# MisterBourbaki/vector-quantization-by-ml

Measured on NVIDIA B200. Metric: vq_lookups_per_sec, higher is better.
Workload: dtype f16

## Files before the change

### vector-quantization-by-ml_b200/csrc/common.cuh

```cuda
#pragma once

#include <cuda_bf16.h>
#include <cuda_fp16.h>
#include <cuda_runtime.h>
#include <stdint.h>
#include <stdio.h>

#include "../../include/vqb.h"

namespace vqb {

void set_error(const char* fmt, ...);

#define VQB_CUDA_TRY(expr)                                                              \
  do {                                                                                  \
    cudaError_t _e = (expr);                                                            \
    if (_e != cudaSuccess) {                                                            \
      vqb::set_error("%s:%d: %s -> %s", __FILE__, __LINE__, #expr, cudaGetErrorString(_e)); \
      return VQB_ERR_CUDA;                                                              \
    }                                                                                   \
  } while (0)

#define VQB_REQUIRE(cond, code, ...)                                                    \
  do {                                                                                  \
// ... 136 lines not shown
#pragma unroll
  for (int i = 0; i < 4; ++i) {
    const float2 f = __half22float2(*reinterpret_cast<const __half2*>(&w[i]));
    o.v[2 * i] = f.x; o.v[2 * i + 1] = f.y;
  }
  return o;
}

template <typename T> struct Raw8 { uint4 r; };
template <> struct Raw8<float> { float4 a, b; };
template <typename T> __device__ __forceinline__ Raw8<T> load_raw8(const T* p) {
  Raw8<T> o; o.r = __ldg(reinterpret_cast<const uint4*>(p)); return o;
}
template <> __device__ __forceinline__ Raw8<float> load_raw8<float>(const float* p) {
  Raw8<float> o;
  o.a = __ldg(reinterpret_cast<const float4*>(p));
  o.b = __ldg(reinterpret_cast<const float4*>(p) + 1);
  return o;
}
__device__ __forceinline__ F8 raw_to_f8(const Raw8<float>& w) {
  F8 o; o.v[0] = w.a.x; o.v[1] = w.a.y; o.v[2] = w.a.z; o.v[3] = w.a.w; o.v[4] = w.b.x; o.v[5] = w.b.y; o.v[6] = w.b.z; o.v[7] = w.b.w;
  return o;
}
__device__ __forceinline__ F8 raw_to_f8(const Raw8<__nv_bfloat16>& w) {
  F8 o;
  o.v[0] = __uint_as_float(w.r.x << 16); o.v[1] = __uint_as_float(w.r.x & 0xffff0000u);
  o.v[2] = __uint_as_float(w.r.y << 16); o.v[3] = __uint_as_float(w.r.y & 0xffff0000u);
  o.v[4] = __uint_as_float(w.r.z << 16); o.v[5] = __uint_as_float(w.r.z & 0xffff0000u);
  o.v[6] = __uint_as_float(w.r.w << 16); o.v[7] = __uint_as_float(w.r.w & 0xffff0000u);
  return o;
}
__device__ __forceinline__ F8 raw_to_f8(const Raw8<__half>& w) {
  const uint32_t u[4] = {w.r.x, w.r.y, w.r.z, w.r.w};
  F8 o;
#pragma unroll
  for (int i = 0; i < 4; ++i) {
    const float2 f = __half22float2(*reinterpret_cast<const __half2*>(&u[i]));
    o.v[2 * i] = f.x; o.v[2 * i + 1] = f.y;
  }
  return o;
}

__device__ __forceinline__ float warp_sum(float v) {
#pragma unroll
  for (int o = 16; o > 0; o >>= 1) v += __shfl_xor_sync(0xffffffffu, v, o);
  return v;
}
__device__ __forceinline__ double warp_sum(double v) {
#pragma unroll
  for (int o = 16; o > 0; o >>= 1) v += __shfl_xor_sync(0xffffffffu, v, o);
  return v;
}

#define VQB_DISPATCH_DTYPE(dtype, T, ...)                                                    \
  switch (dtype) {                                                                           \
    case VQB_F32:  { using T = float;          __VA_ARGS__; break; }                          \
    case VQB_BF16: { using T = __nv_bfloat16;  __VA_ARGS__; break; }                          \
    case VQB_F16:  { using T = __half;         __VA_ARGS__; break; }                          \
    default: vqb::set_error("unknown latent dtype %d", (int)(dtype)); return VQB_ERR_INVALID; \
  }

inline int dtype_size(int dt) { return dt == VQB_F32 ? 4 : 2; }

int launch_prepare_latents(const void* x, int x_dtype, int64_t rows, int64_t rows_per_head, int d, int dp,
                           const float* chdr, __half* xb, float* xinv, float* xn2, __half* xaug, uint32_t* scal,
                           cudaStream_t st);
int launch_make_bias(const void* cache, const CacheLayout& CL, int64_t H, int K, int metric,
                     uint32_t* scal, float* bias, float* err, __half* caug, cudaStream_t st, int derive_dx_dp = 0);
int launch_sample_bound(const void* x, int x_dtype, int64_t rows, int d, uint32_t* scal, cudaStream_t st);
struct ConvArgs {
  const void* x = nullptr;
  int x_dtype = 0;
  int d = 0;
};
int launch_search_tc(const __half* xb, const float* xinv, const float* xn2, float tie, const __half* xaug,
                     const __half* cb, const __half* caug, const float* chdr, const float* bias, int aug_mode,
                     int64_t H, int64_t N, int K, int dp, void* cand, uint32_t* scal, bool timing, cudaStream_t st,
                     const ConvArgs& conv = ConvArgs());
int search_tc_aug_mode(int64_t N, int K, int metric);
int search_tc_conv_ok(int64_t N, int K, int d, int x_dtype, int aug_mode, int requested);

int launch_loss_finalize(const double* part, const long long* cntp, int nblocks, int d, float* loss_out,
                         cudaStream_t st);

__device__ __forceinline__ float clamp_row_scale(float& s, float two_q, float two_mq) {
  const float cap = 32768.f * two_q;
  if (s > cap) s = cap;
  const float a = s * two_mq;
  return a >= 5.9604645e-8f ? a : 0.f;
}

constexpr float kTieSlack = 5.0e-7f;
__device__ __forceinline__ float row_norm2_bound(float n2, float r2) {
  return (n2 + 2.f * sqrtf(n2 * r2) + r2) * 1.0001f;
}

constexpr float kSampleGuard = 1.125f;
__device__ __forceinline__ float dx_bound_16bit(float xmax, int dp, float two_mq) {
  const float inv_s = fmaxf(xmax * 1.220703125e-4f, two_mq * 3.0517578125e-5f);
  return sqrtf((float)dp) * 2.9802322e-8f * inv_s * 1.01f;
}

__device__ __forceinline__ float pow2_scale_bits(float m) {
  const uint32_t ef = (__float_as_uint(m) >> 23) & 0xffu;
  if (!(m > 0.f) || ef == 0xffu) return 1.f;
  int sh = 14 - ((int)ef - 126);
  if (sh > 100) sh = 100;
  if (sh < -100) sh = -100;
  return __uint_as_float((uint32_t)(127 + sh) << 23);
}
__device__ __forceinline__ float pow2_recip(float s) { return __uint_as_float(0x7F000000u - __float_as_uint(s)); }

__host__ __device__ inline float pow2_scale(float m) {
  if (!(m > 0.f) || !isfinite(m)) return 1.f;
  int e = ilogbf(m) + 1;
  int sh = 14 - e;
  if (sh > 100) sh = 100;
  if (sh < -100) sh = -100;
  return ldexpf(1.f, sh);
}

}
```

### vector-quantization-by-ml_b200/csrc/ema.cu

```cuda
#include "common.cuh"

namespace vqb {

constexpr int kChunkRows = 64;

struct EmaLayout {
  size_t off_counts;
  size_t off_cursor;
  size_t off_start;
  size_t off_scale;
  size_t off_acc;
  size_t zero_bytes;
  size_t off_sorted;
  size_t off_total;
  size_t off_table;
  size_t total;
};
constexpr int kSortBlocks = 148;
constexpr int kSortMaxK = 12288;
inline EmaLayout ema_layout(int64_t H, int64_t N, int K, int d) {
  EmaLayout L;
  size_t o = 0;
  L.off_counts = o; o += align_up((size_t)H * K * 4);
  L.off_cursor = o; o += align_up((size_t)H * K * 4);
// ... 34 lines not shown

__global__ void ema_hist_kernel(const int64_t* __restrict__ idx, const uint8_t* __restrict__ mask, int64_t N, int K,
                                uint32_t* __restrict__ counts) {
  const int h = blockIdx.y;
  const int64_t n = (int64_t)blockIdx.x * blockDim.x + threadIdx.x;
  if (n >= N) return;
  if (mask && !mask[n]) return;
  const int64_t k = idx[(int64_t)h * N + n];
  if (k >= 0 && k < K) atomicAdd(counts + (int64_t)h * K + k, 1u);
}

__global__ void ema_scan_kernel(const uint32_t* __restrict__ counts, int K, uint32_t* __restrict__ start) {
  const int h = blockIdx.x;
  const uint32_t* c = counts + (int64_t)h * K;
  uint32_t* s = start + (int64_t)h * (K + 1);
  __shared__ uint32_t wsum[32];
  __shared__ uint32_t carry;
  if (threadIdx.x == 0) carry = 0;
  __syncthreads();
  const int lane = threadIdx.x & 31, warp = threadIdx.x >> 5;
  for (int base = 0; base < K; base += 1024) {
    const int k = base + threadIdx.x;
    const uint32_t v = k < K ? c[k] : 0u;
    uint32_t inc = v;
#pragma unroll
    for (int o = 1; o < 32; o <<= 1) {
      const uint32_t t = __shfl_up_sync(0xffffffffu, inc, o);
      if (lane >= o) inc += t;
    }
    if (lane == 31) wsum[warp] = inc;
    __syncthreads();
    if (warp == 0) {
      uint32_t w = wsum[lane];
#pragma unroll
      for (int o = 1; o < 32; o <<= 1) {
        const uint32_t t = __shfl_up_sync(0xffffffffu, w, o);
        if (lane >= o) w += t;
      }
      wsum[lane] = w;
    }
    __syncthreads();
    const uint32_t before = carry + (warp ? wsum[warp - 1] : 0u) + inc - v;
    if (k < K) s[k] = before;
    __syncthreads();
    if (threadIdx.x == 1023) carry = before + v;
    __syncthreads();
  }
  if (threadIdx.x == 0) s[K] = carry;
}

__global__ void ema_place_kernel(const int64_t* __restrict__ idx, const uint8_t* __restrict__ mask, int64_t N, int K,
                                 const uint32_t* __restrict__ start, uint32_t* __restrict__ cursor,
                                 int* __restrict__ sorted) {
  const int h = blockIdx.y;
  const int64_t n = (int64_t)blockIdx.x * blockDim.x + threadIdx.x;
  if (n >= N) return;
  if (mask && !mask[n]) return;
  const int64_t k = idx[(int64_t)h * N + n];
  if (k < 0 || k >= K) return;
  const uint32_t pos = start[(int64_t)h * (K + 1) + k] + atomicAdd(cursor + (int64_t)h * K + k, 1u);
  sorted[(int64_t)h * N + pos] = (int)n;
}


__global__ void __launch_bounds__(1024)
sort_hist_kernel(const int64_t* __restrict__ idx, const uint8_t* __restrict__ mask, int64_t N, int K,
                 uint32_t* __restrict__ table) {
  extern __shared__ uint32_t s_cnt[];
  const int h = blockIdx.y, b = blockIdx.x, B = gridDim.x;
  for (int k = threadIdx.x; k < K; k += blockDim.x) s_cnt[k] = 0u;
  __syncthreads();
  const int64_t span = (N + B - 1) / B, r0 = (int64_t)b * span, r1 = r0 + span < N ? r0 + span : N;
  for (int64_t n = r0 + threadIdx.x; n < r1; n += blockDim.x) {
    if (mask && !mask[n]) continue;
    const int64_t k = idx[(int64_t)h * N + n];
    if (k >= 0 && k < K) atomicAdd(s_cnt + k, 1u);
  }
  __syncthreads();
  uint32_t* t = table + ((int64_t)h * B + b) * K;
  for (int k = threadIdx.x; k < K; k += blockDim.x) t[k] = s_cnt[k];
}

__global__ void __launch_bounds__(256)
sort_prefix_kernel(uint32_t* __restrict__ table, int B, int K, uint32_t* __restrict__ counts) {
  const int h = blockIdx.y;
  const int k = blockIdx.x * blockDim.x + threadIdx.x;
  if (k >= K) return;
  uint32_t* t = table + (int64_t)h * B * K + k;
  uint32_t v = 0u;
  int b = 0;
  for (; b + 8 <= B; b += 8) {
    uint32_t x[8];
#pragma unroll
    for (int u = 0; u < 8; ++u) x[u] = t[(int64_t)(b + u) * K];
#pragma unroll
    for (int u = 0; u < 8; ++u) { t[(int64_t)(b + u) * K] = v; v += x[u]; }
  }
  for (; b < B; ++b) { const uint32_t x = t[(int64_t)b * K]; t[(int64_t)b * K] = v; v += x; }
  counts[(int64_t)h * K + k] = v;
}

__global__ void __launch_bounds__(1024)
sort_place_kernel(const int64_t* __restrict__ idx, const uint8_t* __restrict__ mask, int64_t N, int K,
                  const uint32_t* __restrict__ start, const uint32_t* __restrict__ table, int* __restrict__ sorted) {
  extern __shared__ uint32_t s_cur[];
  const int h = blockIdx.y, b = blockIdx.x, B = gridDim.x;
  const uint32_t* t = table + ((int64_t)h * B + b) * K;
  const uint32_t* st = start + (int64_t)h * (K + 1);
  for (int k = threadIdx.x; k < K; k += blockDim.x) s_cur[k] = st[k] + t[k];
  __syncthreads();
  const int64_t span = (N + B - 1) / B, r0 = (int64_t)b * span, r1 = r0 + span < N ? r0 + span : N;
  for (int64_t n = r0 + threadIdx.x; n < r1; n += blockDim.x) {
    if (mask && !mask[n]) continue;
    const int64_t k = idx[(int64_t)h * N + n];
    if (k < 0 || k >= K) continue;
    sorted[(int64_t)h * N + atomicAdd(s_cur + k, 1u)] = (int)n;
  }
}

static int launch_code_sort(const int64_t* idx, const uint8_t* mask, int64_t H, int64_t N, int K, uint32_t* counts,
                            uint32_t* cursor, uint32_t* start, int* sorted, uint32_t* table, cudaStream_t st) {
  if (K <= kSortMaxK && table != nullptr && N >= 4096) {
    const dim3 g((unsigned)kSortBlocks, (unsigned)H);
    const size_t smem = (size_t)K * 4;
    sort_hist_kernel<<<g, 1024, smem, st>>>(idx, mask, N, K, table);
    VQB_LAUNCH_CHECK();
    sort_prefix_kernel<<<dim3((unsigned)((K + 255) / 256), (unsigned)H), 256, 0, st>>>(table, kSortBlocks, K, counts);
    VQB_LAUNCH_CHECK();
    ema_scan_kernel<<<(unsigned)H, 1024, 0, st>>>(counts, K, start);
    VQB_LAUNCH_CHECK();
    sort_place_kernel<<<g, 1024, smem, st>>>(idx, mask, N, K, start, table, sorted);
    VQB_LAUNCH_CHECK();
    return VQB_OK;
  }
  dim3 g1((unsigned)((N + 255) / 256), (unsigned)H);
  ema_hist_kernel<<<g1, 256, 0, st>>>(idx, mask, N, K, counts);
  VQB_LAUNCH_CHECK();
  ema_scan_kernel<<<(unsigned)H, 1024, 0, st>>>(counts, K, start);
  VQB_LAUNCH_CHECK();
  ema_place_kernel<<<g1, 256, 0, st>>>(idx, mask, N, K, start, cursor, sorted);
  VQB_LAUNCH_CHECK();
  return VQB_OK;
}

template <typename T>
__global__ void __launch_bounds__(256, 3)
ema_segsum_kernel(const T* __restrict__ x, const int64_t* __restrict__ idx, const int* __restrict__ sorted,
                  const uint32_t* __restrict__ start, int64_t N, int K, int d, const int* __restrict__ scale_p,
                  unsigned long long* __restrict__ acc) {
  const int h = blockIdx.y;
  const int lane = threadIdx.x & 31;
  const int64_t chunk = (int64_t)blockIdx.x * (blockDim.x >> 5) + (threadIdx.x >> 5);
  const int64_t total = start[(int64_t)h * (K + 1) + K];
  const int64_t p0 = chunk * kChunkRows;
  if (p0 >= total) return;
  const int64_t p1 = p0 + kChunkRows < total ? p0 + kChunkRows : total;
  const float scale = ldexpf(1.f, scale_p[0]);
  const T* xh = x + (int64_t)h * N * d;
  const int64_t* idxh = idx + (int64_t)h * N;
  const int* srt = sorted + (int64_t)h * N;
  unsigned long long* acch = acc + (int64_t)h * K * d;
  const bool vec = (d & 3) == 0;

  const int n = (int)(p1 - p0);
  const int r_lo = lane < n ? srt[p0 + lane] : 0;
  const int r_hi = lane + 32 < n ? srt[p0 + 32 + lane] : 0;
  const int k_lo = lane < n ? (int)idxh[r_lo] : -1;
  const int k_hi = lane + 32 < n ? (int)idxh[r_hi] : -1;

  if ((d & 7) == 0) {
    for (int c0 = 0; c0 < d; c0 += 256) {
      const int j = c0 + lane * 8;
      const bool on = j < d;
      long long a[8];
#pragma unroll
      for (int e = 0; e < 8; ++e) a[e] = 0;
      int cur = -1;
      for (int i0 = 0; i0 < n; i0 += 4) {
        F8 v[4];
        int kk[4];
#pragma unroll
        for (int u = 0; u < 4; ++u) {
          const int i = i0 + u;
          const int r = __shfl_sync(0xffffffffu, i < 32 ? r_lo : r_hi, i & 31);
          kk[u] = __shfl_sync(0xffffffffu, i < 32 ? k_lo : k_hi, i & 31);
          if (i < n && on) v[u] = load8<T>(xh + (int64_t)r * d + j);
          else {
#pragma unroll
            for (int e = 0; e < 8; ++e) v[u].v[e] = 0.f;
          }
        }
#pragma unroll
        for (int u = 0; u < 4; ++u) {
          if (i0 + u < n) {
            if (kk[u] != cur) {
              if (cur >= 0 && on) {
                unsigned long long* o = acch + (int64_t)cur * d + j;
#pragma unroll
                for (int e = 0; e < 8; ++e) if (a[e]) atomicAdd(o + e, (unsigned long long)a[e]);
              }
#pragma unroll
              for (int e = 0; e < 8; ++e) a[e] = 0;
              cur = kk[u];
            }
#pragma unroll
            for (int e = 0; e < 8; ++e) a[e] += __float2ll_rn(v[u].v[e] * scale);
          }
        }
      }
      if (cur >= 0 && on) {
        unsigned long long* o = acch + (int64_t)cur * d + j;
#pragma unroll
        for (int e = 0; e < 8; ++e) if (a[e]) atomicAdd(o + e, (unsigned long long)a[e]);
      }
    }
    return;
  }

  for (int c0 = 0; c0 < d; c0 += 128) {
    const int j = c0 + lane * 4;
    const bool on = j < d;
    long long a0 = 0, a1 = 0, a2 = 0, a3 = 0;
    int cur = -1;
    for (int i0 = 0; i0 < n; i0 += 4) {
      float4 v[4];
      int kk[4];
#pragma unroll
      for (int u = 0; u < 4; ++u) {
        const int i = i0 + u;
        const int r = __shfl_sync(0xffffffffu, i < 32 ? r_lo : r_hi, i & 31);
        kk[u] = __shfl_sync(0xffffffffu, i < 32 ? k_lo : k_hi, i & 31);
        v[u] = make_float4(0.f, 0.f, 0.f, 0.f);
        if (i < n && on) {
          const T* xr = xh + (int64_t)r * d + j;
          if (vec) v[u] = load4<T>(xr);
          else {
            v[u].x = to_f32<T>(xr[0]);
            v[u].y = j + 1 < d ? to_f32<T>(xr[1]) : 0.f;
            v[u].z = j + 2 < d ? to_f32<T>(xr[2]) : 0.f;
            v[u].w = j + 3 < d ? to_f32<T>(xr[3]) : 0.f;
          }
        }
      }
#pragma unroll
      for (int u = 0; u < 4; ++u) {
        if (i0 + u < n) {
          if (kk[u] != cur) {
            if (cur >= 0 && on) {
              unsigned long long* o = acch + (int64_t)cur * d + j;
              if (a0) atomicAdd(o + 0, (unsigned long long)a0);
              if (j + 1 < d && a1) atomicAdd(o + 1, (unsigned long long)a1);
              if (j + 2 < d && a2) atomicAdd(o + 2, (unsigned long long)a2);
              if (j + 3 < d && a3) atomicAdd(o + 3, (unsigned long long)a3);
            }
            a0 = a1 = a2 = a3 = 0;
            cur = kk[u];
          }
          a0 += __float2ll_rn(v[u].x * scale);
          a1 += __float2ll_rn(v[u].y * scale);
          a2 += __float2ll_rn(v[u].z * scale);
          a3 += __float2ll_rn(v[u].w * scale);
        }
      }
    }
    if (cur >= 0 && on) {
      unsigned long long* o = acch + (int64_t)cur * d + j;
      if (a0) atomicAdd(o + 0, (unsigned long long)a0);
      if (j + 1 < d && a1) atomicAdd(o + 1, (unsigned long long)a1);
      if (j + 2 < d && a2) atomicAdd(o + 2, (unsigned long long)a2);
      if (j + 3 < d && a3) atomicAdd(o + 3, (unsigned long long)a3);
    }
  }
}

__global__ void ema_finalize_kernel(const long long* __restrict__ acc, const uint32_t* __restrict__ counts,
                                    const int* __restrict__ scale_p, int64_t HK, int d, float* __restrict__ stats) {
  const int64_t i = (int64_t)blockIdx.x * blockDim.x + threadIdx.x;
  const int64_t n = HK * (d + 1);
  if (i >= n) return;
  const int64_t k = i / (d + 1);
  const int j = (int)(i - k * (d + 1));
  if (j == d) stats[i] = (float)counts[k];
  else stats[i] = (float)ldexp((double)acc[k * d + j], -scale_p[0]);
}


struct FusedScale { int s; int pad; int e; int P; };

__global__ void fused_scale_kernel(const float* __restrict__ bound2, const uint32_t* __restrict__ own_bound,
                                   int64_t rows, int two_terms, int* __restrict__ scale) {
  float b = bound2 ? (bound2[0] + bound2[1]) : __uint_as_float(own_bound[0]);
  if (!(b > 0.f) || !isfinite(b)) b = 1.f;
  int e;
  frexpf(b, &e);
  e += 1;
  if (e > 100) e = 100;
  if (e < -100) e = -100;
  int lr = 0;
  while (((int64_t)1 << lr) < rows + 1) ++lr;
  int P = 22;
  if (two_terms) { P = 62 - lr; if (P > 44) P = 44; }
  scale[0] = P - e;
  scale[2] = e;
  scale[3] = P;
}


constexpr int kFusedChunkRows = 128;

struct RvqExtra {
  float* out;
  float* res_out;
  float* q_level;
  __half* next_xb;
  float* next_xinv;
  float* next_xn2;
  __half* next_xaug;
  uint32_t* next_scal;
  const float* next_chdr;
  int first;
  int dp;
};

template <typename T, int NB, int TERMS, bool RVQ>
__global__ void __launch_bounds__(256, 2)
quantize_ema_kernel(const T* __restrict__ x, const float* __restrict__ cb, const int64_t* __restrict__ idx,
                    const int* __restrict__ sorted, const uint32_t* __restrict__ start, int64_t N, int K, int d,
                    int training, const int* __restrict__ scale_p, float* __restrict__ q,
                    float* __restrict__ loss_rows, unsigned long long* __restrict__ acc, const RvqExtra R) {
  constexpr int U0 = (sizeof(T) == 2 ? 8 : 4) / NB;
  constexpr int U = RVQ ? (U0 > 1 ? U0 / 2 : 1) : U0;
  const int h = blockIdx.y;
  const int lane = threadIdx.x & 31;
  const int64_t chunk = (int64_t)blockIdx.x * (blockDim.x >> 5) + (threadIdx.x >> 5);
  const int64_t total = start[(int64_t)h * (K + 1) + K];
  const int64_t p0 = chunk * kFusedChunkRows;
  if (p0 >= total) return;
  const int n = (int)((p0 + kFusedChunkRows < total ? p0 + kFusedChunkRows : total) - p0);
  const int lpr = NB == 1 ? d >> 3 : 32;
  const int rpi = 32 / lpr;
  const int grp = lane / lpr, gl = lane - grp * lpr;
  const int j = gl * 8;
  const int e = scale_p[2], P = scale_p[3];
  const float M1 = ldexpf(1.5f, e + 1);
  const float M2 = ldexpf(1.5f, e + 23 - P);
  const uint32_t M1b = __float_as_uint(M1), M2b = __float_as_uint(M2);
  const int shift = P - 22;
  const T* xh = x + (int64_t)h * N * d;
  const float* cbh = cb + (int64_t)h * K * d;
  const int64_t* idxh = idx + (int64_t)h * N;
  const int* srt = sorted + (int64_t)h * N;
  float* qh = q + (int64_t)h * N * d;
  unsigned long long* acch = acc + (int64_t)h * K * d;

  int rid[4], kid[4];
#pragma unroll
  for (int t = 0; t < 4; ++t) {
    rid[t] = lane + 32 * t < n ? srt[p0 + 32 * t + lane] : 0;
    kid[t] = lane + 32 * t < n ? (int)idxh[rid[t]] : -1;
  }

  uint32_t sh[NB][8], sl[NB][8];
  float c[NB][8];
#pragma unroll
  for (int b = 0; b < NB; ++b)
#pragma unroll
    for (int t = 0; t < 8; ++t) { sh[b][t] = 0u; sl[b][t] = 0u; c[b][t] = 0.f; }
  int cur = -1;
  uint32_t cnt = 0;
  float max_n2 = 0.f, max_r2 = 0.f;
// ... 86 lines not shown
              const float4 p0 = *reinterpret_cast<const float4*>(R.out + off), p1 = *(reinterpret_cast<const float4*>(R.out + off) + 1);
              const float pv[8] = {p0.x, p0.y, p0.z, p0.w, p1.x, p1.y, p1.z, p1.w};
#pragma unroll
              for (int t = 0; t < 8; ++t) acc8[t] = __fadd_rn(pv[t], o[t]);
            }
            *reinterpret_cast<float4*>(R.out + off) = make_float4(acc8[0], acc8[1], acc8[2], acc8[3]);
            *(reinterpret_cast<float4*>(R.out + off) + 1) = make_float4(acc8[4], acc8[5], acc8[6], acc8[7]);
            }
#pragma unroll
            for (int t = 0; t < 8; ++t) {
              rn[b].v[t] = __fsub_rn(v.v[t], o[t]);
              mabs = fmaxf(mabs, fabsf(rn[b].v[t]));
            }
            *reinterpret_cast<float4*>(R.res_out + off) = make_float4(rn[b].v[0], rn[b].v[1], rn[b].v[2], rn[b].v[3]);
            *(reinterpret_cast<float4*>(R.res_out + off) + 1) = make_float4(rn[b].v[4], rn[b].v[5], rn[b].v[6], rn[b].v[7]);
            if (R.q_level) {
              *reinterpret_cast<float4*>(R.q_level + off) = make_float4(o[0], o[1], o[2], o[3]);
              *(reinterpret_cast<float4*>(R.q_level + off) + 1) = make_float4(o[4], o[5], o[6], o[7]);
            }
          }
        }
      }
      if (RVQ && R.next_xb) {
        const bool live = kk[u] >= 0;
        for (int o2 = lpr >> 1; o2 > 0; o2 >>= 1) mabs = fmaxf(mabs, __shfl_xor_sync(0xffffffffu, mabs, o2));
        float s = pow2_scale_bits(mabs);
        const float a = clamp_row_scale(s, R.next_chdr[4], R.next_chdr[5]);
        const float is = pow2_recip(s);
        if (gl == 0 && live) {
          R.next_xinv[rr[u]] = a > 0.f ? is : -is;
          const uint32_t aa = (uint32_t)__half_as_ushort(__float2half_rn(a));
          *reinterpret_cast<uint4*>(R.next_xaug + (int64_t)rr[u] * 8) = make_uint4(aa | (aa << 16), aa, 0u, 0u);
        }
        float n2 = 0.f, r2 = 0.f;
#pragma unroll
        for (int b = 0; b < NB; ++b) {
          uint32_t pk[4];
#pragma unroll
          for (int t = 0; t < 4; ++t) {
            const float v0 = rn[b].v[2 * t], v1 = rn[b].v[2 * t + 1];
            const __half2 hh = __floats2half2_rn(v0 * s, v1 * s);
            const float2 f = __half22float2(hh);
            pk[t] = *reinterpret_cast<const uint32_t*>(&hh);
            const float b0 = f.x * is, b1 = f.y * is;
            n2 += b0 * b0 + b1 * b1;
            const float e0 = v0 - b0, e1 = v1 - b1;
            r2 += e0 * e0 + e1 * e1;
          }
          if (live)
            *reinterpret_cast<uint4*>(R.next_xb + (int64_t)rr[u] * R.dp + b * 256 + j) = make_uint4(pk[0], pk[1], pk[2], pk[3]);
        }
        for (int o2 = lpr >> 1; o2 > 0; o2 >>= 1) {
          n2 += __shfl_xor_sync(0xffffffffu, n2, o2);
          r2 += __shfl_xor_sync(0xffffffffu, r2, o2);
        }
        if (gl == 0 && live) R.next_xn2[rr[u]] = row_norm2_bound(n2, r2);
        max_n2 = fmaxf(max_n2, n2);
        max_r2 = fmaxf(max_r2, r2);
      }
      if (loss_rows) {
        for (int o2 = lpr >> 1; o2 > 0; o2 >>= 1) sq += __shfl_xor_sync(0xffffffffu, sq, o2);
        if (kk[u] >= 0 && gl == 0) loss_rows[(int64_t)h * N + rr[u]] = sq;
      }
    }
  }
  flush();
  if (RVQ && R.next_xb) {
#pragma unroll
    for (int o2 = 16; o2 > 0; o2 >>= 1) {
      max_n2 = fmaxf(max_n2, __shfl_xor_sync(0xffffffffu, max_n2, o2));
      max_r2 = fmaxf(max_r2, __shfl_xor_sync(0xffffffffu, max_r2, o2));
    }
    if (lane == 0) {
      const float infl = 1.f + (float)R.dp * 2.4e-7f;
      atomicMax(R.next_scal + 0, __float_as_uint(sqrtf(max_n2 * infl) * 1.00001f));
      atomicMax(R.next_scal + 1, __float_as_uint(sqrtf(max_r2 * infl) * 1.00001f));
      if (blockIdx.x == 0 && threadIdx.x == 0) R.next_scal[7] = __float_as_uint(R.next_chdr[4]);
    }
  }
}

__global__ void __launch_bounds__(256)
loss_rows_partial_kernel(const float* __restrict__ loss_rows, int64_t rows, int64_t span, double* __restrict__ part,
                         long long* __restrict__ cntp) {
  const int64_t r0 = (int64_t)blockIdx.x * span;
  const int64_t r1 = r0 + span < rows ? r0 + span : rows;
  double t = 0.0;
  for (int64_t r = r0 + threadIdx.x; r < r1; r += 256) t += (double)loss_rows[r];
  __shared__ double s[256];
  s[threadIdx.x] = t;
  __syncthreads();
  for (int o = 128; o > 0; o >>= 1) {
    if ((int)threadIdx.x < o) s[threadIdx.x] += s[threadIdx.x + o];
    __syncthreads();
  }
  if (threadIdx.x == 0) { part[blockIdx.x] = s[0]; cntp[blockIdx.x] = r1 > r0 ? r1 - r0 : 0; }
}

constexpr int kLossBlocks = 1024;
struct FusedLayout {
  EmaLayout E;
  size_t off_loss_rows;
  size_t off_part;
  size_t off_cnt;
  size_t total;
};
inline FusedLayout fused_layout(int64_t H, int64_t N, int K, int d) {
  FusedLayout L;
  L.E = ema_layout(H, N, K, d);
  size_t o = L.E.total;
  L.off_loss_rows = o; o += align_up((size_t)(H * N > 0 ? H * N : 1) * 4);
  L.off_part = o;      o += align_up((size_t)kLossBlocks * 8);
  L.off_cnt = o;       o += align_up((size_t)kLossBlocks * 8);
  L.total = o;
  return L;
}
inline bool fused_width_ok(int d) { return d == 512 || (d >= 8 && d <= 256 && (d & (d - 1)) == 0); }


constexpr int kMomentRows = 256;
template <typename T>
__global__ void __launch_bounds__(256)
column_moments_kernel(const T* __restrict__ x, const uint8_t* __restrict__ mask, int64_t N, int d,
                      double* __restrict__ out, long long* __restrict__ rows_used) {
  const int h = blockIdx.y;
  const int64_t r0 = (int64_t)blockIdx.x * kMomentRows;
  const int64_t r1 = r0 + kMomentRows < N ? r0 + kMomentRows : N;
  const T* xh = x + (int64_t)h * N * d;
  for (int c = threadIdx.x; c < d; c += blockDim.x) {
    double s = 0.0, ss = 0.0;
    for (int64_t r = r0; r < r1; ++r) {
      if (mask && !mask[r]) continue;
      const double v = (double)to_f32<T>(xh[r * d + c]);
      s += v;
      ss = fma(v, v, ss);
    }
    atomicAdd(out + ((int64_t)h * d + c) * 2, s);
    atomicAdd(out + ((int64_t)h * d + c) * 2 + 1, ss);
  }
  if (threadIdx.x == 0) {
    long long n = 0;
    for (int64_t r = r0; r < r1; ++r) n += (!mask || mask[r]) ? 1 : 0;
    atomicAdd(reinterpret_cast<unsigned long long*>(rows_used + h), (unsigned long long)n);
  }
}

__device__ __forceinline__ float torch_lerp(float a, float b, float w) {
  const float diff = b - a;
  return fabsf(w) < 0.5f ? fmaf(w, diff, a) : fmaf(w - 1.f, diff, b);
}

__global__ void ema_apply_counts_kernel(const float* __restrict__ stats, float* __restrict__ cluster_size, float w,
                                        int K, int d, float* __restrict__ total) {
  const int h = blockIdx.x;
  __shared__ double s[1024];
  double t = 0.0;
  for (int k = threadIdx.x; k < K; k += 1024) {
    const int64_t i = (int64_t)h * K + k;
    const float v = torch_lerp(cluster_size[i], stats[i * (d + 1) + d], w);
    cluster_size[i] = v;
    t += (double)v;
  }
  s[threadIdx.x] = t;
  __syncthreads();
  for (int o = 512; o > 0; o >>= 1) {
    if ((int)threadIdx.x < o) s[threadIdx.x] += s[threadIdx.x + o];
    __syncthreads();
  }
  if (threadIdx.x == 0) total[h] = (float)s[0];
}

__global__ void __launch_bounds__(256)
ema_apply_rows_kernel(const float* __restrict__ stats, const float* __restrict__ cluster_size,
                      float* __restrict__ embed_avg, float* __restrict__ embeddings, float w, float eps, float keps,
                      int l2, int64_t H, int K, int d, const float* __restrict__ total) {
  const int lane = threadIdx.x & 31;
  const int64_t row = (int64_t)blockIdx.x * (blockDim.x >> 5) + (threadIdx.x >> 5);
  if (row >= H * K) return;
  const int64_t h = row / K;
// ... 155 lines not shown
  return VQB_OK;
}

extern "C" int vqb_quantize_ema_supported(int d) { return fused_width_ok(d) ? 1 : 0; }

extern "C" size_t vqb_quantize_ema_workspace_bytes(int64_t H, int64_t N, int K, int d) {
  if (H <= 0 || N < 0 || K <= 0 || d <= 0) return 0;
  return fused_layout(H, N, K, d).total;
}

static int quantize_ema_impl(const void* x, int x_dtype, const float* codebook, const int64_t* idx,
                             const float* absmax_bound2, int training, int want_loss, float* q_out,
                             float* loss_out, float* stats, int64_t H, int64_t N, int K, int d, void* ws,
                             size_t ws_bytes, const RvqExtra* rvq, void* stream) {
  VQB_REQUIRE(x && codebook && idx && (q_out || rvq) && stats && ws, VQB_ERR_INVALID, "vqb_quantize_ema: null pointer");
  VQB_REQUIRE(H > 0 && N >= 0 && K > 0 && d > 0 && H < 65536, VQB_ERR_INVALID, "vqb_quantize_ema: bad shape");
  VQB_REQUIRE(N < (1ll << 31), VQB_ERR_UNSUPPORTED, "N must be < 2^31");
  VQB_REQUIRE(fused_width_ok(d), VQB_ERR_UNSUPPORTED, "vqb_quantize_ema: d=%d (need a power of two <= 256, or 512)", d);
  VQB_REQUIRE(!want_loss || loss_out, VQB_ERR_INVALID, "vqb_quantize_ema: loss_out is null");
  FusedLayout L = fused_layout(H, N, K, d);
  VQB_REQUIRE(ws_bytes >= L.total, VQB_ERR_WORKSPACE, "quantize_ema workspace too small: %zu < %zu", ws_bytes, L.total);
  cudaStream_t st = (cudaStream_t)stream;
  char* w = (char*)ws;
  uint32_t* counts = (uint32_t*)(w + L.E.off_counts);
  uint32_t* cursor = (uint32_t*)(w + L.E.off_cursor);
  uint32_t* start = (uint32_t*)(w + L.E.off_start);
  int* scale = (int*)(w + L.E.off_scale);
  long long* acc = (long long*)(w + L.E.off_acc);
  int* sorted = (int*)(w + L.E.off_sorted);
  float* loss_rows = want_loss ? (float*)(w + L.off_loss_rows) : nullptr;
  double* part = (double*)(w + L.off_part);
  long long* cntp = (long long*)(w + L.off_cnt);
  const int two_terms = x_dtype == VQB_F32 ? 1 : 0;
  VQB_CUDA_TRY(cudaMemsetAsync(w, 0, L.E.zero_bytes, st));
  if (N > 0) {
    if (!absmax_bound2) {
      VQB_DISPATCH_DTYPE(x_dtype, T,
        absmax_kernel<T><<<1184, 256, 0, st>>>((const T*)x, H * N * (int64_t)d, (uint32_t*)(scale + 1)));
      VQB_LAUNCH_CHECK();
    }
    fused_scale_kernel<<<1, 1, 0, st>>>(absmax_bound2, (const uint32_t*)(scale + 1), N, two_terms, scale);
    VQB_LAUNCH_CHECK();
    if (rvq && rvq->next_scal) VQB_CUDA_TRY(cudaMemsetAsync(rvq->next_scal, 0, 8, st));
    if (int rc = launch_code_sort(idx, nullptr, H, N, K, counts, cursor, start, sorted,
                                  K <= kSortMaxK ? (uint32_t*)(w + L.E.off_table) : nullptr, st)) return rc;
    const int64_t chunks = (N + kFusedChunkRows - 1) / kFusedChunkRows;
    dim3 g2((unsigned)((chunks + 7) / 8), (unsigned)H);
#define VQB_QE_LAUNCH(T, NB, TERMS)                                                                          \
    quantize_ema_kernel<T, NB, TERMS, false><<<g2, 256, 0, st>>>((const T*)x, codebook, idx, sorted, start, N, K, d, \
                                                                 training, scale, q_out, loss_rows,              \
                                                                 (unsigned long long*)acc, RvqExtra{})
    if (rvq) {
      if (d == 512)
        quantize_ema_kernel<float, 2, 2, true><<<g2, 256, 0, st>>>((const float*)x, codebook, idx, sorted, start, N, K, d,
                                                                   training, scale, nullptr, loss_rows,
                                                                   (unsigned long long*)acc, *rvq);
      else
        quantize_ema_kernel<float, 1, 2, true><<<g2, 256, 0, st>>>((const float*)x, codebook, idx, sorted, start, N, K, d,
                                                                   training, scale, nullptr, loss_rows,
                                                                   (unsigned long long*)acc, *rvq);
    } else if (d == 512) {
      if (x_dtype == VQB_F32) VQB_QE_LAUNCH(float, 2, 2);
      else if (x_dtype == VQB_BF16) VQB_QE_LAUNCH(__nv_bfloat16, 2, 1);
      else if (x_dtype == VQB_F16) VQB_QE_LAUNCH(__half, 2, 1);
      else { set_error("unknown latent dtype %d", x_dtype); return VQB_ERR_INVALID; }
    } else {
      if (x_dtype == VQB_F32) VQB_QE_LAUNCH(float, 1, 2);
      else if (x_dtype == VQB_BF16) VQB_QE_LAUNCH(__nv_bfloat16, 1, 1);
      else if (x_dtype == VQB_F16) VQB_QE_LAUNCH(__half, 1, 1);
      else { set_error("unknown latent dtype %d", x_dtype); return VQB_ERR_INVALID; }
    }
#undef VQB_QE_LAUNCH
    VQB_LAUNCH_CHECK();
  }
  const int64_t n = H * (int64_t)K * (d + 1);
  ema_finalize_kernel<<<(unsigned)((n + 255) / 256), 256, 0, st>>>(acc, counts, scale, H * (int64_t)K, d, stats);
  VQB_LAUNCH_CHECK();
  if (want_loss) {
    const int64_t rows = H * N;
    int nblocks = 0;
    if (rows > 0) {
      const int64_t span = (rows + kLossBlocks - 1) / kLossBlocks;
      nblocks = (int)((rows + span - 1) / span);
      loss_rows_partial_kernel<<<nblocks, 256, 0, st>>>(loss_rows, rows, span, part, cntp);
      VQB_LAUNCH_CHECK();
    }
    int rc = launch_loss_finalize(part, cntp, nblocks, d, loss_out, st);
    if (rc) return rc;
  }
  return VQB_OK;
}

extern "C" int vqb_quantize_ema(const void* x, int x_dtype, const float* codebook, const int64_t* idx,
                                const float* absmax_bound2, int training, int want_loss, float* q_out,
                                float* loss_out, float* stats, int64_t H, int64_t N, int K, int d, void* ws,
                                size_t ws_bytes, void* stream) {
  return quantize_ema_impl(x, x_dtype, codebook, idx, absmax_bound2, training, want_loss, q_out, loss_out, stats, H, N,
                           K, d, ws, ws_bytes, nullptr, stream);
}

extern "C" int vqb_rvq_level_ema_supported(int d) { return (d == 64 || d == 128 || d == 256 || d == 512) ? 1 : 0; }

extern "C" int vqb_rvq_level_ema(const float* residual_in, float* residual_out, const float* codebook,
                                 const int64_t* idx, const float* absmax_bound2, int training, int first_level,
                                 float* quantized_out, float* q_out, float* loss_out, float* stats, int64_t N, int K,
                                 int d, void* ws, size_t ws_bytes, void* next_ws, size_t next_ws_bytes,
                                 const void* next_cache, void* stream) {
  VQB_REQUIRE(residual_in && residual_out && loss_out, VQB_ERR_INVALID, "vqb_rvq_level_ema: null pointer");
  VQB_REQUIRE(vqb_rvq_level_ema_supported(d), VQB_ERR_UNSUPPORTED, "vqb_rvq_level_ema: d=%d (64, 128, 256 or 512)", d);
  VQB_REQUIRE(residual_in != residual_out, VQB_ERR_INVALID, "vqb_rvq_level_ema: rows are visited in code order, the "
              "residual cannot be updated in place");
  RvqExtra R = {};
  R.out = quantized_out; R.res_out = residual_out; R.q_level = q_out; R.first = first_level; R.dp = d_pad(d);
  if (next_ws) {
    VQB_REQUIRE(next_cache != nullptr, VQB_ERR_INVALID, "vqb_rvq_level_ema: next_ws needs next_cache");
    SearchLayout SL = search_layout(1, N, K, d);
    VQB_REQUIRE(next_ws_bytes >= SL.total, VQB_ERR_WORKSPACE, "next-level search workspace too small");
    R.next_xb = (__half*)((char*)next_ws + SL.off_xb);
    R.next_xaug = (__half*)((char*)next_ws + SL.off_xaug);
    R.next_xinv = (float*)((char*)next_ws + SL.off_xinv);
    R.next_xn2 = (float*)((char*)next_ws + SL.off_xn2);
    R.next_scal = (uint32_t*)((char*)next_ws + SL.off_scal);
    R.next_chdr = (const float*)((const char*)next_cache + cache_layout(1, K, d).off_hdr);
  }
  return quantize_ema_impl(residual_in, VQB_F32, codebook, idx, absmax_bound2, training, 1, nullptr, loss_out, stats, 1,
                           N, K, d, ws, ws_bytes, &R, stream);
}

extern "C" int vqb_ema_apply_counts(const float* stats, float* cluster_size, float weight, int64_t H, int K, int d,
                                    float* totals_out, void* stream) {
  VQB_REQUIRE(stats && cluster_size && totals_out, VQB_ERR_INVALID, "vqb_ema_apply_counts: null pointer");
  VQB_REQUIRE(H > 0 && K > 0 && d > 0, VQB_ERR_INVALID, "vqb_ema_apply_counts: bad shape");
  ema_apply_counts_kernel<<<(unsigned)H, 1024, 0, (cudaStream_t)stream>>>(stats, cluster_size, weight, K, d, totals_out);
  VQB_LAUNCH_CHECK();
  return VQB_OK;
}

extern "C" int vqb_ema_apply_rows(const float* stats, const float* cluster_size, float* embed_avg, float* embeddings,
                                  float weight, double eps, int64_t k_total, int l2norm, int64_t H, int K, int d,
                                  const float* totals, void* stream) {
  VQB_REQUIRE(stats && cluster_size && embed_avg && embeddings && totals, VQB_ERR_INVALID,
              "vqb_ema_apply_rows: null pointer");
  VQB_REQUIRE(H > 0 && K > 0 && d > 0 && k_total >= K, VQB_ERR_INVALID, "vqb_ema_apply_rows: bad shape");
  const int64_t rows = H * (int64_t)K;
  ema_apply_rows_kernel<<<(unsigned)((rows + 7) / 8), 256, 0, (cudaStream_t)stream>>>(
      stats, cluster_size, embed_avg, embeddings, weight, (float)eps, (float)((double)k_total * eps), l2norm, H, K, d,
      totals);
  VQB_LAUNCH_CHECK();
  return VQB_OK;
}

extern "C" int vqb_ema_apply(const float* stats, float* cluster_size, float* embed_avg, float* embeddings,
                             float weight, double eps, int l2norm, int64_t H, int K, int d, void* ws,
                             size_t ws_bytes, void* stream) {
  VQB_REQUIRE(ws != nullptr && ws_bytes >= (size_t)H * 4, VQB_ERR_WORKSPACE, "ema_apply workspace too small");
  int rc = vqb_ema_apply_counts(stats, cluster_size, weight, H, K, d, (float*)ws, stream);
  if (rc) return rc;
  return vqb_ema_apply_rows(stats, cluster_size, embed_avg, embeddings, weight, eps, K, l2norm, H, K, d,
                            (const float*)ws, stream);
}

extern "C" int vqb_expire_scatter(const void* x, int x_dtype, const int64_t* sample_rows, int64_t m, float threshold,
                                  float reset, int l2norm, float* cluster_size, float* embed_avg, float* embeddings,
                                  int64_t N, int K, int d, void* stream) {
  VQB_REQUIRE(x && cluster_size && embed_avg && embeddings, VQB_ERR_INVALID, "vqb_expire_scatter: null pointer");
  VQB_REQUIRE(m >= 0 && N > 0 && K > 0 && d > 0, VQB_ERR_INVALID, "vqb_expire_scatter: bad shape");
  if (m == 0) return VQB_OK;
  VQB_REQUIRE(sample_rows != nullptr, VQB_ERR_INVALID, "vqb_expire_scatter: sample_rows is null");
  VQB_DISPATCH_DTYPE(x_dtype, T,
    expire_scatter_kernel<T><<<1, 1024, 0, (cudaStream_t)stream>>>((const T*)x, sample_rows, m, threshold, reset,
                                                                  l2norm, cluster_size, embed_avg, embeddings, N, K, d));
// ... 36 lines not shown
```

### vector-quantization-by-ml_b200/csrc/gather.cu

```cuda
#include "common.cuh"

namespace vqb {

constexpr int kGatherThreads = 256;

struct GatherLayout {
  size_t off_part;
  size_t off_cnt;
  size_t total;
};
static int gather_grid(int64_t rows) {
  static int sms = 0;
  if (!sms) {
    int dev = 0;
    cudaGetDevice(&dev);
    cudaDeviceGetAttribute(&sms, cudaDevAttrMultiProcessorCount, dev);
    if (sms <= 0) sms = 148;
  }
  int64_t need = (rows + (kGatherThreads / 32) - 1) / (kGatherThreads / 32);
  int64_t cap = (int64_t)sms * 8;
  return (int)(need < cap ? (need > 0 ? need : 1) : cap);
}
static GatherLayout gather_layout() {
  GatherLayout L;
// ... 53 lines not shown
        if (kLoss) { sq = fmaf(df.x, df.x, sq); sq = fmaf(df.y, df.y, sq); sq = fmaf(df.z, df.z, sq); sq = fmaf(df.w, df.w, sq); }
      }
    } else {
      for (int j = lane; j < d; j += 32) {
        const float xv = to_f32<T>(xr[j]);
        const float cv = cr[j];
        const float df = __fsub_rn(cv, xv);
        qr[j] = training ? __fadd_rn(xv, df) : cv;
        if (kLoss) sq = fmaf(df, df, sq);
      }
    }
    if (kLoss && in_loss) { sqd += (double)sq; if (lane == 0) ++used; }
  }
  if (kLoss) {
    sqd = warp_sum(sqd);
    __shared__ double s_sq[kGatherThreads / 32];
    __shared__ long long s_n[kGatherThreads / 32];
    if (lane == 0) { s_sq[warp] = sqd; s_n[warp] = used; }
    __syncthreads();
    if (threadIdx.x == 0) {
      double t = 0.0;
      long long c = 0;
      for (int i = 0; i < wpb; ++i) { t += s_sq[i]; c += s_n[i]; }
      part[blockIdx.x] = t;
      cntp[blockIdx.x] = c;
    }
  }
}

template <typename T, bool kLoss>
__global__ void __launch_bounds__(kGatherThreads)
gather_st_loss_narrow_kernel(const T* __restrict__ x, const float* __restrict__ cb, const int64_t* __restrict__ idx,
                             const uint8_t* __restrict__ mask, int training, float* __restrict__ q, int64_t H,
                             int64_t N, int K, int d, double* __restrict__ part, long long* __restrict__ cntp) {
  const int lane = threadIdx.x & 31, warp = threadIdx.x >> 5;
  const int wpb = kGatherThreads / 32;
  const int lpr = d >> 3, rpi = 32 / lpr;
  const int grp = lane / lpr, j = (lane - grp * lpr) * 8;
  const int64_t rows = H * N;
  double sqd = 0.0;
  long long used = 0;
  for (int64_t row0 = ((int64_t)blockIdx.x * wpb + warp) * rpi; row0 < rows; row0 += (int64_t)gridDim.x * wpb * rpi) {
    const int64_t row = row0 + grp;
    if (row >= rows) continue;
    const int64_t h = row / N, n = row - h * N;
    const int64_t code = idx[row];
    const bool in_loss = mask == nullptr || mask[n] != 0;
    const F8 xv = load8<T>(x + row * (int64_t)d + j);
    const float* cr = cb + (h * K + code) * (int64_t)d + j;
    const float4 c0 = __ldg(reinterpret_cast<const float4*>(cr)), c1 = __ldg(reinterpret_cast<const float4*>(cr) + 1);
    const float cv[8] = {c0.x, c0.y, c0.z, c0.w, c1.x, c1.y, c1.z, c1.w};
    float o[8], sq = 0.f;
#pragma unroll
    for (int e = 0; e < 8; ++e) {
      const float df = __fsub_rn(cv[e], xv.v[e]);
      o[e] = training ? __fadd_rn(xv.v[e], df) : cv[e];
      if (kLoss) sq = fmaf(df, df, sq);
    }
    float* qr = q + row * (int64_t)d + j;
    __stcs(reinterpret_cast<float4*>(qr), make_float4(o[0], o[1], o[2], o[3]));
    __stcs(reinterpret_cast<float4*>(qr) + 1, make_float4(o[4], o[5], o[6], o[7]));
    if (kLoss && in_loss) { sqd += (double)sq; if (j == 0) ++used; }
  }
  if (kLoss) {
    sqd = warp_sum(sqd);
#pragma unroll
    for (int o2 = 16; o2 > 0; o2 >>= 1) used += __shfl_xor_sync(0xffffffffu, used, o2);
    __shared__ double s_sq[kGatherThreads / 32];
    __shared__ long long s_n[kGatherThreads / 32];
    if (lane == 0) { s_sq[warp] = sqd; s_n[warp] = used; }
    __syncthreads();
    if (threadIdx.x == 0) {
      double t = 0.0;
      long long c = 0;
      for (int i = 0; i < wpb; ++i) { t += s_sq[i]; c += s_n[i]; }
      part[blockIdx.x] = t;
      cntp[blockIdx.x] = c;
    }
  }
}

__global__ void loss_finalize_kernel(const double* __restrict__ part, const long long* __restrict__ cntp, int nblocks,
                                     int d, float* __restrict__ loss_out) {
  __shared__ double s[256];
  __shared__ long long c[256];
  double t = 0.0;
  long long n = 0;
  for (int i = threadIdx.x; i < nblocks; i += 256) { t += part[i]; n += cntp[i]; }
  s[threadIdx.x] = t;
  c[threadIdx.x] = n;
  __syncthreads();
  for (int o = 128; o > 0; o >>= 1) {
    if ((int)threadIdx.x < o) { s[threadIdx.x] += s[threadIdx.x + o]; c[threadIdx.x] += c[threadIdx.x + o]; }
    __syncthreads();
  }
  if (threadIdx.x == 0) {
    const double denom = (double)c[0] * (double)d;
    loss_out[0] = denom > 0.0 ? (float)(s[0] / denom) : __int_as_float(0x7fc00000);
    loss_out[1] = (float)c[0];
  }
}

struct RotCoef {
  float sx, sc;
  float rx, rc;
  float lam;
  float a;
  float b;
};
__device__ __forceinline__ RotCoef rot_scales(double nx2, double nc2) {
  const double nc = sqrt(nc2), sx = fmax(sqrt(nx2), 1e-6);
  RotCoef r;
  r.sx = (float)sx;
  r.sc = (float)fmax(nc, 1e-6);
  r.rx = __frcp_rn(r.sx);
  r.rc = __frcp_rn(r.sc);
  r.lam = (float)(nc / sx);
  r.a = r.b = 0.f;
  return r;
}
__device__ __forceinline__ float rot_div(float v, float s, float r) {
  const float q0 = __fmul_rn(v, r);
  return fmaf(fmaf(-q0, s, v), r, q0);
}
__device__ __forceinline__ void rot_finish(RotCoef& r, float gx, float gc, float nw2) {
  const float nw = fmaxf(sqrtf(nw2), 1e-12f), rnw = __frcp_rn(nw);
  const float gq = rot_div(gc, r.sc, r.rc);
  const float gw = rot_div(__fadd_rn(rot_div(gx, r.sx, r.rx), gq), nw, rnw);
  r.a = nw2 > 0.f ? -2.f * r.lam * rot_div(gw, nw, rnw) : 0.f;
  r.b = 2.f * r.lam * gq;
}
__device__ __forceinline__ float rot_u(float xv, const RotCoef& r) { return rot_div(xv, r.sx, r.rx); }
__device__ __forceinline__ float rot_sum(float xv, float cv, const RotCoef& r) {
  return __fadd_rn(rot_div(xv, r.sx, r.rx), rot_div(cv, r.sc, r.rc));
}

template <typename T, bool kRot>
__global__ void __launch_bounds__(kGatherThreads)
st_commit_backward_kernel(const float* __restrict__ gq, const float* __restrict__ gl, const T* __restrict__ x,
                          const float* __restrict__ cb, const int64_t* __restrict__ idx,
                          const uint8_t* __restrict__ mask, float coef, float* __restrict__ gx, int64_t H, int64_t N,
                          int K, int d) {
  const int lane = threadIdx.x & 31, warp = threadIdx.x >> 5;
  const int wpb = kGatherThreads / 32;
  const int64_t rows = H * N;
  const float s = coef * gl[0];
  for (int64_t row = (int64_t)blockIdx.x * wpb + warp; row < rows; row += (int64_t)gridDim.x * wpb) {
    const int64_t h = row / N, n = row - h * N;
    const bool in_loss = mask == nullptr || mask[n] != 0;
    const float sc = in_loss ? s : 0.f;
    const T* xr = x + row * (int64_t)d;
    const float* cr = cb + (h * K + idx[row]) * (int64_t)d;
    const float* gr = gq + row * (int64_t)d;
    float* o = gx + row * (int64_t)d;
    if (!kRot || !in_loss) {
      for (int j = lane; j < d; j += 32) o[j] = fmaf(sc, to_f32<T>(xr[j]) - cr[j], gr[j]);
      continue;
    }
    double nx2 = 0.0, nc2 = 0.0;
    float gdx = 0.f, gdc = 0.f;
    for (int j = lane; j < d; j += 32) {
      const float xv = to_f32<T>(xr[j]), cv = cr[j], g = gr[j];
      nx2 = fma((double)xv, (double)xv, nx2);
      nc2 = fma((double)cv, (double)cv, nc2);
      gdx = fmaf(g, xv, gdx);
      gdc = fmaf(g, cv, gdc);
    }
    RotCoef rc = rot_scales(warp_sum(nx2), warp_sum(nc2));
    float nw2 = 0.f;
    for (int j = lane; j < d; j += 32) {
      const float e = rot_sum(to_f32<T>(xr[j]), cr[j], rc);
      nw2 = fmaf(e, e, nw2);
    }
    rot_finish(rc, warp_sum(gdx), warp_sum(gdc), warp_sum(nw2));
    for (int j = lane; j < d; j += 32) {
      const float xv = to_f32<T>(xr[j]), cv = cr[j];
      o[j] = fmaf(sc, xv - cv, fmaf(rc.b, rot_u(xv, rc), fmaf(rc.a, rot_sum(xv, cv, rc), rc.lam * gr[j])));
    }
  }
}

__global__ void __launch_bounds__(kGatherThreads)
rvq_level_kernel(const float* res_in, float* res_out, const float* __restrict__ cb, const int64_t* __restrict__ idx,
// ... 532 lines not shown
```

Measured before the change: 264.2 million.

## Fold code-sort scan and loss finalize into last-block-done kernels

Merges the separate exclusive-scan kernel into the sort prefix kernel: each block scans its tile of counts, and the last block to finish (found through an atomic counter in scratch) adds the per-block offsets. The loss finalize launch is likewise folded into the partial-loss kernel through a last-block atomic. Both remove kernel launches and their serialization gaps, at the cost of threadfence and atomic overhead, a serial offset loop in one thread, and a dependence on the counters in scratch being zeroed.

```diff
diff --git a/vector-quantization-by-ml_b200/csrc/common.cuh b/vector-quantization-by-ml_b200/csrc/common.cuh
--- a/vector-quantization-by-ml_b200/csrc/common.cuh
+++ b/vector-quantization-by-ml_b200/csrc/common.cuh
@@ -242,6 +242,26 @@
 
 int launch_loss_finalize(const double* part, const long long* cntp, int nblocks, int d, float* loss_out,
                          cudaStream_t st);
+__device__ __forceinline__ void loss_finalize_block(const double* part, const long long* cntp, int nblocks, int d,
+                                                    float* loss_out) {
+  __shared__ double s[256];
+  __shared__ long long c[256];
+  double t = 0.0;
+  long long n = 0;
+  for (int i = threadIdx.x; i < nblocks; i += 256) { t += __ldcg(part + i); n += __ldcg(cntp + i); }
+  s[threadIdx.x] = t;
+  c[threadIdx.x] = n;
+  __syncthreads();
+  for (int o = 128; o > 0; o >>= 1) {
+    if ((int)threadIdx.x < o) { s[threadIdx.x] += s[threadIdx.x + o]; c[threadIdx.x] += c[threadIdx.x + o]; }
+    __syncthreads();
+  }
+  if (threadIdx.x == 0) {
+    const double denom = (double)c[0] * (double)d;
+    loss_out[0] = denom > 0.0 ? (float)(s[0] / denom) : __int_as_float(0x7fc00000);
+    loss_out[1] = (float)c[0];
+  }
+}
 
 __device__ __forceinline__ float clamp_row_scale(float& s, float two_q, float two_mq) {
   const float cap = 32768.f * two_q;
diff --git a/vector-quantization-by-ml_b200/csrc/ema.cu b/vector-quantization-by-ml_b200/csrc/ema.cu
--- a/vector-quantization-by-ml_b200/csrc/ema.cu
+++ b/vector-quantization-by-ml_b200/csrc/ema.cu
@@ -140,22 +140,55 @@
 }
 
 __global__ void __launch_bounds__(256)
-sort_prefix_kernel(uint32_t* __restrict__ table, int B, int K, uint32_t* __restrict__ counts) {
+sort_prefix_kernel(uint32_t* __restrict__ table, int B, int K, uint32_t* __restrict__ counts,
+                   uint32_t* __restrict__ start, uint32_t* __restrict__ scratch) {
   const int h = blockIdx.y;
   const int k = blockIdx.x * blockDim.x + threadIdx.x;
-  if (k >= K) return;
-  uint32_t* t = table + (int64_t)h * B * K + k;
   uint32_t v = 0u;
-  int b = 0;
-  for (; b + 8 <= B; b += 8) {
-    uint32_t x[8];
-#pragma unroll
-    for (int u = 0; u < 8; ++u) x[u] = t[(int64_t)(b + u) * K];
-#pragma unroll
-    for (int u = 0; u < 8; ++u) { t[(int64_t)(b + u) * K] = v; v += x[u]; }
-  }
-  for (; b < B; ++b) { const uint32_t x = t[(int64_t)b * K]; t[(int64_t)b * K] = v; v += x; }
-  counts[(int64_t)h * K + k] = v;
+  if (k < K) {
+    uint32_t* t = table + (int64_t)h * B * K + k;
+    int b = 0;
+    for (; b + 8 <= B; b += 8) {
+      uint32_t x[8];
+#pragma unroll
+      for (int u = 0; u < 8; ++u) x[u] = t[(int64_t)(b + u) * K];
+#pragma unroll
+      for (int u = 0; u < 8; ++u) { t[(int64_t)(b + u) * K] = v; v += x[u]; }
+    }
+    for (; b < B; ++b) { const uint32_t x = t[(int64_t)b * K]; t[(int64_t)b * K] = v; v += x; }
+    counts[(int64_t)h * K + k] = v;
+  }
+  __shared__ uint32_t wsum[8];
+  __shared__ bool last;
+  const int lane = threadIdx.x & 31, warp = threadIdx.x >> 5;
+  uint32_t inc = v;
+#pragma unroll
+  for (int o = 1; o < 32; o <<= 1) {
+    const uint32_t x = __shfl_up_sync(0xffffffffu, inc, o);
+    if (lane >= o) inc += x;
+  }
+  if (lane == 31) wsum[warp] = inc;
+  __syncthreads();
+  uint32_t before = inc - v;
+  for (int w = 0; w < warp; ++w) before += wsum[w];
+  uint32_t* st = start + (int64_t)h * (K + 1);
+  uint32_t* sc = scratch + (int64_t)h * K;
+  if (k < K) st[k] = before;
+  if (threadIdx.x == 255) sc[1 + blockIdx.x] = before + v;
+  __threadfence();
+  __syncthreads();
+  if (threadIdx.x == 0) last = atomicAdd(sc, 1u) == gridDim.x - 1;
+  __syncthreads();
+  if (!last) return;
+  __shared__ uint32_t off[kSortMaxK / 256 + 1];
+  if (threadIdx.x == 0) {
+    uint32_t o = 0u;
+    for (int x = 0; x < (int)gridDim.x; ++x) { off[x] = o; o += __ldcg(sc + 1 + x); }
+    st[K] = o;
+  }
+  __syncthreads();
+  for (int j = threadIdx.x; j < K; j += 256)
+    if (j >> 8) st[j] = __ldcg(st + j) + off[j >> 8];
 }
 
 __global__ void __launch_bounds__(1024)
@@ -178,14 +211,13 @@
 
 static int launch_code_sort(const int64_t* idx, const uint8_t* mask, int64_t H, int64_t N, int K, uint32_t* counts,
                             uint32_t* cursor, uint32_t* start, int* sorted, uint32_t* table, cudaStream_t st) {
-  if (K <= kSortMaxK && table != nullptr && N >= 4096) {
+  if (K >= 2 && K <= kSortMaxK && table != nullptr && N >= 4096) {
     const dim3 g((unsigned)kSortBlocks, (unsigned)H);
     const size_t smem = (size_t)K * 4;
     sort_hist_kernel<<<g, 1024, smem, st>>>(idx, mask, N, K, table);
     VQB_LAUNCH_CHECK();
-    sort_prefix_kernel<<<dim3((unsigned)((K + 255) / 256), (unsigned)H), 256, 0, st>>>(table, kSortBlocks, K, counts);
-    VQB_LAUNCH_CHECK();
-    ema_scan_kernel<<<(unsigned)H, 1024, 0, st>>>(counts, K, start);
+    sort_prefix_kernel<<<dim3((unsigned)((K + 255) / 256), (unsigned)H), 256, 0, st>>>(table, kSortBlocks, K, counts,
+                                                                                       start, cursor);
     VQB_LAUNCH_CHECK();
     sort_place_kernel<<<g, 1024, smem, st>>>(idx, mask, N, K, start, table, sorted);
     VQB_LAUNCH_CHECK();
@@ -344,6 +376,7 @@
 
 
 struct FusedScale { int s; int pad; int e; int P; };
+constexpr int kLossDone = 8;
 
 __global__ void fused_scale_kernel(const float* __restrict__ bound2, const uint32_t* __restrict__ own_bound,
                                    int64_t rows, int two_terms, int* __restrict__ scale) {
@@ -596,19 +629,28 @@
 
 __global__ void __launch_bounds__(256)
 loss_rows_partial_kernel(const float* __restrict__ loss_rows, int64_t rows, int64_t span, double* __restrict__ part,
-                         long long* __restrict__ cntp) {
+                         long long* __restrict__ cntp, unsigned int* __restrict__ done, int d,
+                         float* __restrict__ loss_out) {
   const int64_t r0 = (int64_t)blockIdx.x * span;
   const int64_t r1 = r0 + span < rows ? r0 + span : rows;
   double t = 0.0;
   for (int64_t r = r0 + threadIdx.x; r < r1; r += 256) t += (double)loss_rows[r];
   __shared__ double s[256];
+  __shared__ bool last;
   s[threadIdx.x] = t;
   __syncthreads();
   for (int o = 128; o > 0; o >>= 1) {
     if ((int)threadIdx.x < o) s[threadIdx.x] += s[threadIdx.x + o];
     __syncthreads();
   }
-  if (threadIdx.x == 0) { part[blockIdx.x] = s[0]; cntp[blockIdx.x] = r1 > r0 ? r1 - r0 : 0; }
+  if (threadIdx.x == 0) {
+    part[blockIdx.x] = s[0];
+    cntp[blockIdx.x] = r1 > r0 ? r1 - r0 : 0;
+    __threadfence();
+    last = atomicAdd(done, 1u) == gridDim.x - 1;
+  }
+  __syncthreads();
+  if (last) loss_finalize_block(part, cntp, gridDim.x, d, loss_out);
 }
 
 constexpr int kLossBlocks = 1024;
@@ -930,11 +972,12 @@
     if (rows > 0) {
       const int64_t span = (rows + kLossBlocks - 1) / kLossBlocks;
       nblocks = (int)((rows + span - 1) / span);
-      loss_rows_partial_kernel<<<nblocks, 256, 0, st>>>(loss_rows, rows, span, part, cntp);
+      loss_rows_partial_kernel<<<nblocks, 256, 0, st>>>(loss_rows, rows, span, part, cntp,
+                                                         (unsigned int*)(scale + kLossDone), d, loss_out);
       VQB_LAUNCH_CHECK();
-    }
-    int rc = launch_loss_finalize(part, cntp, nblocks, d, loss_out, st);
-    if (rc) return rc;
+    } else if (int rc = launch_loss_finalize(part, cntp, 0, d, loss_out, st)) {
+      return rc;
+    }
   }
   return VQB_OK;
 }
diff --git a/vector-quantization-by-ml_b200/csrc/gather.cu b/vector-quantization-by-ml_b200/csrc/gather.cu
--- a/vector-quantization-by-ml_b200/csrc/gather.cu
+++ b/vector-quantization-by-ml_b200/csrc/gather.cu
@@ -159,23 +159,7 @@
 
 __global__ void loss_finalize_kernel(const double* __restrict__ part, const long long* __restrict__ cntp, int nblocks,
                                      int d, float* __restrict__ loss_out) {
-  __shared__ double s[256];
-  __shared__ long long c[256];
-  double t = 0.0;
-  long long n = 0;
-  for (int i = threadIdx.x; i < nblocks; i += 256) { t += part[i]; n += cntp[i]; }
-  s[threadIdx.x] = t;
-  c[threadIdx.x] = n;
-  __syncthreads();
-  for (int o = 128; o > 0; o >>= 1) {
-    if ((int)threadIdx.x < o) { s[threadIdx.x] += s[threadIdx.x + o]; c[threadIdx.x] += c[threadIdx.x + o]; }
-    __syncthreads();
-  }
-  if (threadIdx.x == 0) {
-    const double denom = (double)c[0] * (double)d;
-    loss_out[0] = denom > 0.0 ? (float)(s[0] / denom) : __int_as_float(0x7fc00000);
-    loss_out[1] = (float)c[0];
-  }
+  loss_finalize_block(part, cntp, nblocks, d, loss_out);
 }
 
 struct RotCoef {
```

Result: no change. 265.3 million, median of 6 (+0.4%).
